# PlasmaControl/spectrogram-enhancement

Measured on AMD Instinct MI355X. Metric: spectrograms/s (STFT+VAE-denoise fwd) at 1/2/4/8 GPUs; PSNR vs CPU ref, higher is better.
Workload: dtype fp16; 1 GPU; BASELINE config 5 per GPU: end-to-end STFT -> SVD -> autoencoder-denoise inference stream, 16,512-sample fp16 shots -> specgr 128x128 (256 hann / hop 128) -> denoiseSignal default -> 3-layer conv AE (16/32/64, 5x5) fp16 forward -> fp16 reconstructions (32,768 B per shot); shots_per_launch=2048, samples=16512, stft_dtype=fp32, svd_dtype=fp32 (fp64 small algebra), ae_dtype=fp16, parallelism=shot-sharded x1, streams_per_gpu=2

## Files before the change

spectrogram-enhancement_amd/csrc/runtime.hip:

```cpp
#include "runtime.hpp"

#include <algorithm>
#include <atomic>
#include <cstdlib>
#include <cstring>
#include <mutex>
#include <string>

#include "specenh.h"

namespace specenh {
namespace {

struct VariantName {
  const char* name;
  int dflt;
};
constexpr VariantName kVariants[V_COUNT] = {
    {"CONVT_PAIR", 0},      {"PATCH_NO_WL", 0},      {"PATCH_NO_K5", 0},
    {"PATCH_WSPLIT", -1},   {"CONV_NO_S2", 0},       {"CONV_NO_PATCH", 0},
    {"CONV_NO_C1MFMA", 0},  {"CONV_NO_NARROW", 0},   {"WGRAD_GENERIC", 0},
    {"WGRAD_NO_CO1", 0},    {"WGRAD_PERPHASE", 0},   {"SVD_GRAM_TILES", 0},
    {"TAIL_TILES", 0},      {"DECODER_UNFUSED", 0},  {"SVD_NO_TOP1", 0},
    {"CONV_NO_ROWS", 0},    {"CONVT_NO_ROWS", 0},    {"CONV1_NO_ROWS", 0},
    {"ENCODER_UNFUSED", 0},  {"STFT_NO_HOLD", 0},    {"D3_MAP", 0},
    {"ENC2_WPE2", 0},        {"CONVT_SHARED_RING", 0}, {"SVD_RECON_VALU", 0},
    {"ROWS_SHORT_LEAD", 0},  {"SVD_GRAM_F32", 0},
    {"SVD_RECON_BLOCKS", 0}, {"CONVT_PG", 0}, {"SVD_GZ_ROWS", 0}, {"EIG_SPLIT", 0}, {"CO1_VALU", 0},
    {"C1_MASK_MFMA", 1}, {"S2_MIN_NT", 2}, {"PATCH_MIN_WG", 512}, {"WGRAD_WG", 1024}, {"WGRAD_C1_TILES", 4},
    {"EIG_GRID", 32}, {"ROWS_BANDS", -1}, {"CONVT_STORE8", 0},
    {"CONV_ROWS_SCHED", 1}, {"ENC2_SCHED", 1},
};

std::atomic<int> g_variant[V_COUNT];
std::once_flag g_variant_once;

void init_variants() {
  for (int i = 0; i < V_COUNT; ++i) {
    int v = kVariants[i].dflt;
    std::string env = std::string("SPECENH_") + kVariants[i].name;
    if (const char* s = std::getenv(env.c_str()); s && *s) v = std::atoi(s);
    g_variant[i].store(v, std::memory_order_relaxed);
  }
}

int variant_index(const char* name) {
  if (!name) return -1;
  if (std::strncmp(name, "SPECENH_", 8) == 0) name += 8;
  for (int i = 0; i < V_COUNT; ++i)
    if (std::strcmp(name, kVariants[i].name) == 0) return i;
  return -1;
}

constexpr int kMaxDevices = 64;
std::atomic<int> g_cus[kMaxDevices];

constexpr int kRing = 256;
thread_local const void* g_ring[kRing];
thread_local long long g_launches = 0;

thread_local std::string g_last_error;

}

int set_error(int code, const std::string& msg) {
  g_last_error = msg;
  return code;
}

int variant(Variant v) {
  std::call_once(g_variant_once, init_variants);
  return g_variant[v].load(std::memory_order_relaxed);
}

int device_cus() {
  int dev = 0;
  if (hipGetDevice(&dev) != hipSuccess || dev < 0 || dev >= kMaxDevices) return 256;
  int c = g_cus[dev].load(std::memory_order_relaxed);
  if (c > 0) return c;
  if (hipDeviceGetAttribute(&c, hipDeviceAttributeMultiprocessorCount, dev) != hipSuccess || c <= 0)
    c = 256;
  g_cus[dev].store(c, std::memory_order_relaxed);
  return c;
}

hipError_t allow_lds(LdsOptIn& site, std::initializer_list<const void*> kernels, int bytes) {
  static_assert(sizeof(site.done) / sizeof(site.done[0]) == kMaxDevices, "one flag per device");
  int dev = 0;
  hipError_t e = hipGetDevice(&dev);
  if (e != hipSuccess) return e;
  const bool known = dev >= 0 && dev < kMaxDevices;
  if (known && site.done[dev].load(std::memory_order_acquire)) return hipSuccess;
  for (const void* k : kernels) {
    hipFuncAttributes fa{};
    e = hipFuncGetAttributes(&fa, k);
    if (e != hipSuccess) return e;
    e = hipFuncSetAttribute(k, hipFuncAttributeMaxDynamicSharedMemorySize,
                            std::min(bytes, 160 * 1024 - (int)fa.sharedSizeBytes));
    if (e != hipSuccess) return e;
  }
  if (known) site.done[dev].store(true, std::memory_order_release);
  return hipSuccess;
}

hipError_t resident_slots(ResidentSlots& site, const void* kernel, int threads, int lds_bytes,
                          long long* slots) {
  static_assert(sizeof(site.per_cu) / sizeof(site.per_cu[0]) == kMaxDevices, "one count per device");
  int dev = 0;
  hipError_t e = hipGetDevice(&dev);
  if (e != hipSuccess) return e;
  const bool known = dev >= 0 && dev < kMaxDevices;
  int pc = known ? site.per_cu[dev].load(std::memory_order_relaxed) : 0;
  if (pc == 0) {
    e = hipOccupancyMaxActiveBlocksPerMultiprocessor(&pc, kernel, threads, (size_t)lds_bytes);
// ... 83 lines not shown
```

spectrogram-enhancement_amd/csrc/runtime.hpp:

```cpp
#pragma once

#include <hip/hip_runtime.h>

#include <atomic>
#include <initializer_list>
#include <string>

#include "specenh.h"

namespace specenh {

int set_error(int code, const std::string& msg);

inline int ilog2i(int n) {
  int l = 0;
  while ((1 << l) < n) ++l;
  return l;
}

enum Variant : int {
  V_CONVT_PAIR = 0,
  V_PATCH_NO_WL,
  V_PATCH_NO_K5,
  V_PATCH_WSPLIT,
  V_CONV_NO_S2,
  V_CONV_NO_PATCH,
  V_CONV_NO_C1MFMA,
  V_CONV_NO_NARROW,
  V_WGRAD_GENERIC,
  V_WGRAD_NO_CO1,
  V_WGRAD_PERPHASE,
  V_SVD_GRAM_TILES,
  V_TAIL_TILES,
  V_DECODER_UNFUSED,
  V_SVD_NO_TOP1,
  V_CONV_NO_ROWS,
  V_CONVT_NO_ROWS,
  V_CONV1_NO_ROWS,
  V_ENCODER_UNFUSED,
  V_STFT_NO_HOLD,
  V_D3_MAP,
  V_ENC2_WPE2,
  V_CONVT_SHARED_RING,
  V_SVD_RECON_VALU,
  V_ROWS_SHORT_LEAD,
  V_SVD_GRAM_F32,
  V_SVD_RECON_BLOCKS,
  V_CONVT_PG,
  V_SVD_GZ_ROWS,
  V_EIG_SPLIT,
  V_CO1_VALU,
  V_C1_MASK_MFMA,
  V_S2_MIN_NT,
  V_PATCH_MIN_WG,
  V_WGRAD_WG,
  V_WGRAD_C1_TILES,
  V_EIG_GRID,
  V_ROWS_BANDS,
  V_CONVT_STORE8,
  V_CONV_ROWS_SCHED,
  V_ENC2_SCHED,
  V_COUNT
};

int variant(Variant v);

int device_cus();

struct LdsOptIn {
  std::atomic<bool> done[64];
};
hipError_t allow_lds(LdsOptIn& site, std::initializer_list<const void*> kernels, int bytes);

struct ResidentSlots {
  std::atomic<int> per_cu[64];
};
hipError_t resident_slots(ResidentSlots& site, const void* kernel, int threads, int lds_bytes,
                          long long* slots);

template <typename F>
auto with_half_type(int dtype, F&& f) {
  return dtype == SPECENH_DTYPE_F16 ? f(_Float16{}) : f(__bf16{});
}

void note_launch(const void* kernel);

}

#define SPECENH_LAUNCH(K, ...)                                        \
  do {                                                                \
    ::specenh::note_launch(reinterpret_cast<const void*>(&K));        \
    hipLaunchKernelGGL(K, __VA_ARGS__);                               \
  } while (0)
```

spectrogram-enhancement_amd/csrc/svd_denoise.hip:

```cpp
#include <hip/hip_runtime.h>

#include <algorithm>
#include <cmath>
#include <cstdlib>
#include <string>
#include <vector>

#include "fft_common.hpp"
#include "specenh.h"
#include "runtime.hpp"
#include "wave.hpp"

namespace specenh {

typedef float f32x16 __attribute__((ext_vector_type(16)));

struct XView {
  const float* base;
  long long batch_stride;
  long long sk, si;
};

__global__ __launch_bounds__(256) void gram_kernel(XView x, int K, int r, float* G,
                                                   int ntiles_side) {
// ... 1499 lines not shown
      const int klen = RP / KS;
      for (int t = wave; t < 2 * NT * KS; t += 4) {
        const int tile = t % (2 * NT), part = t / (2 * NT);
        const int rt = tile & 1, ct = tile >> 1;
        const float* a_p = sX + (16 * rt + cl) * PX + part * klen + kr;
        const float* b_p = sV + (part * klen + kr) * PV + 16 * ct + cl;
        f4 acc = f4{0.f, 0.f, 0.f, 0.f}, acc2 = f4{0.f, 0.f, 0.f, 0.f};
        int k = 0;
        for (; k + 32 <= klen; k += 32) {
          float av[8], bv[8];
#pragma unroll
          for (int q = 0; q < 8; ++q) {
            av[q] = a_p[k + 4 * q];
            bv[q] = b_p[(k + 4 * q) * PV];
          }
#pragma unroll
          for (int q = 0; q < 8; q += 2) {
            acc = __builtin_amdgcn_mfma_f32_16x16x4f32(av[q], bv[q], acc, 0, 0, 0);
            acc2 = __builtin_amdgcn_mfma_f32_16x16x4f32(av[q + 1], bv[q + 1], acc2, 0, 0, 0);
          }
        }
        for (; k < klen; k += 4)
          acc = __builtin_amdgcn_mfma_f32_16x16x4f32(a_p[k], b_p[k * PV], acc, 0, 0, 0);
        acc += acc2;
        float* yp = sY + part * RB * PY + (16 * rt + 4 * kr) * PY + 16 * ct + cl;
#pragma unroll
        for (int j = 0; j < 4; ++j) yp[j * PY] = acc[j];
      }
    }
    lds_barrier();
    if constexpr (KS == 2) {
      for (int e = tid; e < RB * KPP; e += 256) {
        const int row = e / KPP, c = e % KPP;
        sY[row * PY + c] += sY[RB * PY + row * PY + c];
      }
      lds_barrier();
    }
    for (int t = wave; t < 2 * nit; t += 4) {
      const int rt = t & 1, it = t >> 1;
      const float* y_p = sY + (16 * rt + cl) * PY + kr;
      const float* v_p = sV + (16 * it + cl) * PV + kr;
      f4 acc = f4{0.f, 0.f, 0.f, 0.f};
#pragma unroll
      for (int k = 0; k < KPP; k += 4)
        acc = TRANS ? __builtin_amdgcn_mfma_f32_16x16x4f32(v_p[k], y_p[k], acc, 0, 0, 0)
                    : __builtin_amdgcn_mfma_f32_16x16x4f32(y_p[k], v_p[k], acc, 0, 0, 0);
#pragma unroll
      for (int j = 0; j < 4; ++j) {
        const int row = TRANS ? 16 * rt + cl : 16 * rt + 4 * kr + j;
        const int col = TRANS ? 16 * it + 4 * kr + j : 16 * it + cl;
        if (row < rows && col < r) {
          const float v = complement ? sX[row * PX + col] - acc[j] : acc[j];
          Ob[(long long)(k0 + row) * osk + (long long)col * osi] = to_out<TO>(v);
        }
      }
    }
  };
  fetch(stA, blk0 * RB, min(RB, Kr - blk0 * RB));
  fetch(stB, (blk0 + 1) * RB, blk0 + 1 < blk1 ? min(RB, Kr - (blk0 + 1) * RB) : 0);
  for (int blk = blk0; blk < blk1; blk += 2) {
    block(blk, stA);
    if (blk + 1 < blk1) block(blk + 1, stB);
  }
}

#ifndef SPECENH_TOP1_SWZ
#define SPECENH_TOP1_SWZ 1
#endif
namespace top1 {
constexpr int N = 128;
constexpr int LD = N + 4;
constexpr int MAX_ROUNDS = 24;
constexpr int ZP = SPECENH_TOP1_SWZ ? N + 8 : N;
__host__ __device__ constexpr int zt(int p, int k) {
  return p * ZP + k + (SPECENH_TOP1_SWZ ? 4 * (k >> 6) : 0);
}
__device__ __forceinline__ int ppos(int i) { return SPECENH_TOP1_SWZ ? i ^ ((i >> 3) & 7) : i; }
__device__ __forceinline__ int xz_chunk(int g, int j) {
  if (SPECENH_TOP1_SWZ)
    return 2 * (j >> 1) + (g >> 2) + 4 * ((j & 1) + 2 * ((g >> 1) & 1)) + 16 * (g & 1);
  return 8 * (g & 1) + (g >> 1) + 16 * (j & 1) + 4 * (j >> 1);
}
constexpr size_t LDS_BYTES = (size_t)N * LD * 4 + 4 * ZP * 4 + N * 4 * 4 + 4 * N * 4 * 4 + 64 * 8;

__device__ __forceinline__ void chol4(const double (&M)[4][4], double (&L)[4][4], double (&rinv)[4]) {
#pragma unroll
  for (int j = 0; j < 4; ++j) {
    double d = M[j][j];
#pragma unroll
    for (int l = 0; l < j; ++l) d = fma(-L[j][l], L[j][l], d);
    const bool live = d > 1e-20 * M[j][j] && d > 0.0;
    rinv[j] = live ? rsq64<1>(d) : 0.0;
    L[j][j] = 0.0;
#pragma unroll
    for (int k = j + 1; k < 4; ++k) {
      double s = M[k][j];
#pragma unroll
      for (int l = 0; l < j; ++l) s = fma(-L[k][l], L[j][l], s);
      L[k][j] = s * rinv[j];
      L[j][k] = 0.0;
    }
  }
}

__device__ __forceinline__ void solve_row(const double (&L)[4][4], const double (&rinv)[4],
                                          const double (&y)[4], double (&z)[4]) {
#pragma unroll
  for (int j = 0; j < 4; ++j) {
    double s = y[j];
#pragma unroll
    for (int l = 0; l < j; ++l) s = fma(-z[l], L[j][l], s);
    z[j] = s * rinv[j];
  }
}

__device__ __forceinline__ void jacobi4(float (&A)[4][4], float (&Q)[4][4]) {
#pragma unroll
  for (int a = 0; a < 4; ++a)
#pragma unroll
    for (int b = 0; b < 4; ++b) Q[a][b] = a == b ? 1.f : 0.f;
  for (int sweep = 0; sweep < 6; ++sweep) {
    float off = 0.f, dg = 0.f;
#pragma unroll
    for (int a = 0; a < 4; ++a) {
      dg = fmaf(A[a][a], A[a][a], dg);
#pragma unroll
      for (int b = a + 1; b < 4; ++b) off = fmaf(A[a][b], A[a][b], off);
    }
    if (!(off > 1e-14f * dg)) break;
#pragma unroll
    for (int pr = 0; pr < 6; ++pr) {
      const int p = pr < 3 ? 0 : (pr < 5 ? 1 : 2);
      const int q = pr < 3 ? pr + 1 : (pr < 5 ? pr - 1 : 3);
      const float apq = A[p][q];
      if (apq == 0.f) continue;
      const float tau = 0.5f * (A[q][q] - A[p][p]) * __builtin_amdgcn_rcpf(apq);
      const float t = copysignf(__builtin_amdgcn_rcpf(fabsf(tau) + __builtin_amdgcn_sqrtf(fmaf(tau, tau, 1.f))), tau);
      const float c = __builtin_amdgcn_rsqf(fmaf(t, t, 1.f)), s = t * c;
#pragma unroll
      for (int k = 0; k < 4; ++k) {
        const float akp = A[k][p], akq = A[k][q];
        A[k][p] = c * akp - s * akq;
        A[k][q] = s * akp + c * akq;
        const float qkp = Q[k][p], qkq = Q[k][q];
        Q[k][p] = c * qkp - s * qkq;
        Q[k][q] = s * qkp + c * qkq;
      }
#pragma unroll
      for (int k = 0; k < 4; ++k) {
        const float apk = A[p][k], aqk = A[q][k];
        A[p][k] = c * apk - s * aqk;
        A[q][k] = s * apk + c * aqk;
      }
    }
  }
}

template <int NV>
__device__ __forceinline__ void bsum128(double (&v)[NV], double* sR) {
  const int tid = threadIdx.x, w = tid >> 6;
  if (w < 2) {
#pragma unroll
    for (int j = 0; j < NV; ++j) v[j] = wave_sum_dpp(v[j]);
    if ((tid & 63) == 0)
#pragma unroll
      for (int j = 0; j < NV; ++j) sR[w * NV + j] = v[j];
  }
  lds_barrier();
#pragma unroll
  for (int j = 0; j < NV; ++j) v[j] = sR[j] + sR[NV + j];
}

template <int NV>
__device__ __forceinline__ void gram_sums(const float* sY, const float* sZt, const float* sU,
                                          double* sRed) {
  const int t = threadIdx.x, j = t >> 3, c = t & 7;
  double s = 0.0;
  if (j < NV) {
    const int n = j % 10, src = j / 10;
    const int a = (int)((0x3221110000ULL >> (4 * n)) & 15);
    const int b = (int)((0x3323213210ULL >> (4 * n)) & 15);
#pragma unroll
    for (int i = 0; i < 16; ++i) {
      const int row = SPECENH_TOP1_SWZ ? 8 * i + c : 16 * c + i;
      const float va = src == 0 ? sY[4 * row + a] : (src == 1 ? sZt[zt(a, row)] : sU[4 * row + a]);
      const float vb = src == 0 ? sY[4 * row + b] : (src == 1 ? sZt[zt(b, row)] : sU[4 * row + b]);
      s = fma((double)va, (double)vb, s);
    }
  }
  s += dpp<0xB1, false>(s);
  s += dpp<0x4E, false>(s);
  s += dpp<0x141, false>(s);
  if (c == 0 && j < NV) sRed[j] = s;
  lds_barrier();
}

__device__ __forceinline__ void sym4(const double* p, double (&M)[4][4]) {
  int n = 0;
#pragma unroll
  for (int a = 0; a < 4; ++a)
#pragma unroll
    for (int c = a; c < 4; ++c) {
      M[a][c] = M[c][a] = p[n];
      ++n;
    }
}
}

template <typename TO>
__global__ __launch_bounds__(256, 2) void top1_kernel(XView x, int Kr, int r, float tolv,
                                                       int* flags, TO* out, long long ob,
                                                       long long osk, long long osi,
                                                       long long batch, long long* phase_clk) {
  using namespace top1;
#ifdef SPECENH_TOP1_STATS
  long long tacc[8], tlast;
#define T1_MARK(slot)                                      \
  do {                                                     \
    const long long now_ = __builtin_amdgcn_s_memtime();   \
    tacc[slot] += now_ - tlast;                            \
    tlast = now_;                                          \
  } while (0)
#else
#define T1_MARK(slot) \
  do {                \
  } while (0)
#endif
  extern __shared__ __attribute__((aligned(16))) unsigned char smem[];
  float* sX = reinterpret_cast<float*>(smem);
  float* sZt = sX + N * LD;
  float* sU = sZt + 4 * ZP;
  float* sP = sU + 4 * N;
  double* sR = reinterpret_cast<double*>(sP + 16 * N);
  double* vd = reinterpret_cast<double*>(sP);
  double* ud = vd + N;
  double* hd = ud + N;
  const int tid = threadIdx.x, lane = tid & 63, w = tid >> 6;
#ifdef SPECENH_TOP1_STATS
  for (int q = 0; q < 8; ++q) tacc[q] = 0;
  tlast = __builtin_amdgcn_s_memtime();
#endif
  const long long b = blockIdx.x;
  if (b >= batch) return;
  const float* X = x.base + b * x.batch_stride;

  double fro = 0.0;
  if (x.si == 1) {
    constexpr int NLD = N * N / 4 / 256;
    float4 v[NLD];
#pragma unroll
    for (int u = 0; u < NLD; ++u) {
      const int e = tid + 256 * u, k = e >> 5, i = 4 * (e & 31);
      v[u] = (k < Kr && i < r) ? *reinterpret_cast<const float4*>(X + (long long)k * x.sk + i)
                               : make_float4(0.f, 0.f, 0.f, 0.f);
    }
#pragma unroll
    for (int u = 0; u < NLD; ++u) {
      const int e = tid + 256 * u, k = e >> 5, i = 4 * (e & 31);
      *reinterpret_cast<float4*>(sX + k * LD + i) = v[u];
      fro += (double)v[u].x * v[u].x + (double)v[u].y * v[u].y + (double)v[u].z * v[u].z +
             (double)v[u].w * v[u].w;
    }
  } else {
    for (int e = tid; e < N * N / 4; e += 256) {
      const int i = e >> 5, k = 4 * (e & 31);
      const float4 v = (k < Kr && i < r)
                           ? *reinterpret_cast<const float4*>(X + (long long)i * x.si + k)
                           : make_float4(0.f, 0.f, 0.f, 0.f);
      sX[k * LD + i] = v.x;
// ... 199 lines not shown
    {
      double S[4][4];
      sym4(sR, S);
      chol4(S, L, ri);
    }
    if (tid < N) {
#pragma unroll
      for (int p = 0; p < 4; ++p) yd[p] = y[p];
      solve_row(L, ri, yd, zd);
#pragma unroll
      for (int p = 0; p < 4; ++p) sZt[zt(p, tid)] = (float)zd[p];
    }
    lds_barrier();
    T1_MARK(3);
  }
  auto Xv = [&]() {
    const int k = tid & (N - 1), h = tid >> 7;
    const float* xr = sX + k * LD + 64 * h;
    const double* vv = vd + 64 * h;
    double s0 = 0.0, s1 = 0.0;
#pragma unroll 4
    for (int j = 0; j < 16; ++j) {
      const float4 x4 = *reinterpret_cast<const float4*>(xr + 4 * j);
      const double2 v01 = *reinterpret_cast<const double2*>(vv + 4 * j);
      const double2 v23 = *reinterpret_cast<const double2*>(vv + 4 * j + 2);
      s0 = fma((double)x4.x, v01.x, s0);
      s1 = fma((double)x4.y, v01.y, s1);
      s0 = fma((double)x4.z, v23.x, s0);
      s1 = fma((double)x4.w, v23.y, s1);
    }
    if (h) hd[k] = s0 + s1;
    lds_barrier();
    if (!h) ud[k] = (s0 + s1) + hd[k];
    lds_barrier();
  };
  lds_barrier();
  Xv();
  {
    const int i = tid & (N - 1), h = tid >> 7;
    double s0 = 0.0, s1 = 0.0;
#pragma unroll 8
    for (int kk = 0; kk < 64; kk += 2) {
      const int k = 64 * h + kk;
      s0 = fma((double)sX[k * LD + i], ud[k], s0);
      s1 = fma((double)sX[(k + 1) * LD + i], ud[k + 1], s1);
    }
    if (h) hd[i] = s0 + s1;
    lds_barrier();
    const double w = h ? 0.0 : (s0 + s1) + hd[i];
    double nn[1] = {w * w};
    bsum128<1>(nn, sR + 40);
    if (!h) vd[i] = nn[0] > 0.0 ? w * rsq64<1>(nn[0]) : 0.0;
    lds_barrier();
  }
  Xv();
  T1_MARK(5);
#ifdef SPECENH_TOP1_STATS
  if (flags && tid == 0) flags[b] = bad + 2 * t_used;
#else
  if (flags && tid == 0) flags[b] = bad;
#endif
  TO* Ob = out + b * ob;
  if (osi == 1) {
    for (int e = tid; e < Kr * (r / 4); e += 256) {
      const int k = e / (r / 4), i = 4 * (e % (r / 4));
      const float4 xv = *reinterpret_cast<const float4*>(sX + k * LD + i);
      const double2 v01 = *reinterpret_cast<const double2*>(vd + i);
      const double2 v23 = *reinterpret_cast<const double2*>(vd + i + 2);
      const double u = ud[k];
      TO* o = Ob + (long long)k * osk + i;
      o[0] = to_out<TO>((float)fma(-u, v01.x, (double)xv.x));
      o[1] = to_out<TO>((float)fma(-u, v01.y, (double)xv.y));
      o[2] = to_out<TO>((float)fma(-u, v23.x, (double)xv.z));
      o[3] = to_out<TO>((float)fma(-u, v23.y, (double)xv.w));
    }
  } else {
    for (int e = tid; e < r * (Kr / 4); e += 256) {
      const int i = e / (Kr / 4), k = 4 * (e % (Kr / 4));
      const double vi = vd[i];
      TO* o = Ob + (long long)i * osi + k;
#pragma unroll
      for (int c = 0; c < 4; ++c)
        o[c] = to_out<TO>((float)fma(-ud[k + c], vi, (double)sX[(k + c) * LD + i]));
    }
  }
  T1_MARK(6);
#ifdef SPECENH_TOP1_STATS
  if (phase_clk && tid == 0)
    for (int q = 0; q < 8; ++q) phase_clk[b * 8 + q] = tacc[q];
#endif
#undef T1_MARK
}



__device__ __forceinline__ void gram64_one(XView x, int K, int r, double* G, int nts,
                                           long long b, int tile) {
  __shared__ double sa[16][65], sb[16][65];
  int t = tile, ti = 0;
  while (t >= nts - ti) {
    t -= nts - ti;
    ++ti;
  }
  const int tj = ti + t;
  const float* X = x.base + b * x.batch_stride;
  const int tid = threadIdx.x, tx = tid & 15, ty = tid >> 4;
  double acc[4][4];
#pragma unroll
  for (int i = 0; i < 4; ++i)
#pragma unroll
    for (int j = 0; j < 4; ++j) acc[i][j] = 0.0;
  for (int k0 = 0; k0 < K; k0 += 16) {
    for (int idx = tid; idx < 16 * 64; idx += 256) {
      int kk, c;
      if (x.si == 1) {
        kk = idx >> 6;
        c = idx & 63;
      } else {
        c = idx >> 4;
        kk = idx & 15;
      }
      const int k = k0 + kk, ci = ti * 64 + c, cj = tj * 64 + c;
      sa[kk][c] = (k < K && ci < r) ? (double)X[(long long)k * x.sk + (long long)ci * x.si] : 0.0;
      sb[kk][c] = (k < K && cj < r) ? (double)X[(long long)k * x.sk + (long long)cj * x.si] : 0.0;
    }
    __syncthreads();
#pragma unroll 4
    for (int kk = 0; kk < 16; ++kk) {
      double av[4], bv[4];
#pragma unroll
      for (int i = 0; i < 4; ++i) {
        av[i] = sa[kk][ty * 4 + i];
        bv[i] = sb[kk][tx * 4 + i];
      }
#pragma unroll
      for (int i = 0; i < 4; ++i)
#pragma unroll
        for (int j = 0; j < 4; ++j) acc[i][j] = fma(av[i], bv[j], acc[i][j]);
    }
    __syncthreads();
  }
  double* Gb = G + b * (long long)r * r;
#pragma unroll
  for (int i = 0; i < 4; ++i)
#pragma unroll
    for (int j = 0; j < 4; ++j) {
      const int row = ti * 64 + ty * 4 + i, col = tj * 64 + tx * 4 + j;
      if (row < r && col < r) {
        Gb[(long long)row * r + col] = acc[i][j];
        Gb[(long long)col * r + row] = acc[i][j];
      }
    }
}

__global__ __launch_bounds__(256) void gram64_kernel(XView x, int K, int r, double* G, int nts,
                                                     const int* only, long long nmat) {
  for (long long b = blockIdx.y; b < nmat; b += gridDim.y) {
    if (only && !only[b]) continue;
    gram64_one(x, K, r, G, nts, b, blockIdx.x);
    __syncthreads();
  }
}

__device__ __forceinline__ void tridiag_one(double* G, int n, double* dg, double* eg,
                                            double* taug, long long b) {
  __shared__ double sv[256], sw[256], red[4];
// ... 699 lines not shown
  const EigLayout L = eig_layout(r);
  const long long ch = L.chunk(batch);
  char* w = (char*)workspace;
  double* G64 = (double*)w;
  double* dd = G64 + ch * (long long)r * r;
  double* ee = dd + ch * r;
  double* tau = ee + ch * r;
  double* Z = tau + ch * r;
  double* fac = Z + ch * (long long)r * L.ld;
  int* kinfo = (int*)(fac + 3 * ch * (long long)r * L.ld);
  int* ranges = kinfo + 2 * ch;
  int* num = ranges + 2 * ch;
  double* med = (double*)(((uintptr_t)(num + ch) + 7) & ~(uintptr_t)7);
  const Oriented o = orient(A, m, n, a_stride);
  XView xv = o.xv;
  const int Kr = o.Kr;
  const long long osk = o.osk, osi = o.osi;
  const long long ob = (long long)m * n;
  const size_t osz = dtype_size(odt);
  const int nts64 = (r + 63) / 64, ntri64 = nts64 * (nts64 + 1) / 2;
  const double beta = (double)r / (double)std::max(m, n);
  const double omega = ((0.0 + 0.56 * std::pow(beta, 3.0)) + -0.95 * std::pow(beta, 2.0)) +
                       1.82 * std::pow(beta, 1.0) + 1.43 * std::pow(beta, 0.0);
  for (long long b0 = 0; b0 < batch; b0 += ch) {
    const long long nb = std::min(ch, batch - b0);
    xv.base = A + b0 * a_stride;
    const int* on = only ? only + b0 : nullptr;
    void* ob0 = static_cast<char*>(out) + (size_t)(b0 * ob) * osz;
    const long long gcap = variant(V_EIG_GRID) > 0 ? variant(V_EIG_GRID) : 2LL * device_cus();
    const unsigned gm = on ? (unsigned)std::min<long long>(nb, gcap) : (unsigned)nb;
    const bool merged_fits = (long long)r * Kr <= 128LL * 128;
    if (on && opt_mode < 0 && merged_fits && SPECENH_EIG_MERGED && variant(V_EIG_SPLIT) == 0) {
      const hipError_t e = with_out_type(odt, [&](auto t) {
        return launch_eig_fallback_t<decltype(t)>(xv, Kr, r, G64, nts64, dd, ee, tau, lo, hi, Z,
                                                  fac, L.ld, kinfo, ob0, ob, osk, osi, on, nb, gm,
                                                  st);
      });
      if (e != hipSuccess) return set_error(SPECENH_EHIP, std::string("eigen fallback: ") + hipGetErrorString(e));
      continue;
    }
    SPECENH_LAUNCH(gram64_kernel, dim3(ntri64, gm), dim3(256), 0, st, xv, Kr, r, G64, nts64, on,
                   nb);
    SPECENH_LAUNCH(tridiag_kernel, dim3(gm), dim3(256), 0, st, G64, r, dd, ee, tau, on, nb);
    const int* rg = nullptr;
    if (opt_mode >= 0) {
      SPECENH_LAUNCH(optimal_rank_kernel, dim3((unsigned)nb), dim3(64), 0, st, dd, ee, r,
                         omega, num, med);
      SPECENH_LAUNCH(optimal_ranges_kernel, dim3((unsigned)((nb + 255) / 256)), dim3(256), 0,
                         st, num, nb, r, opt_mode, ranges, bad);
      if (num_out && hipMemcpyAsync(num_out + b0, num, (size_t)nb * 4, hipMemcpyDeviceToDevice,
                                    st) != hipSuccess)
        return set_error(SPECENH_EHIP, "num_sing copy");
      if (med_out && hipMemcpyAsync(med_out + b0, med, (size_t)nb * 8, hipMemcpyDeviceToDevice,
                                    st) != hipSuccess)
        return set_error(SPECENH_EHIP, "median copy");
      rg = ranges;
    }
    SPECENH_LAUNCH(eigvec_kernel, dim3(gm), dim3(256), 0, st, G64, dd, ee, tau, r, lo, hi, rg,
                   Z, fac, L.ld, kinfo, on, nb);
    if (hipGetLastError() != hipSuccess) return set_error(SPECENH_EHIP, "eigen path launch");
    const hipError_t e = with_out_type(odt, [&](auto t) {
      return launch_recon_eig_t<decltype(t)>(xv, Kr, r, Z, L.ld, kinfo, ob0, ob, osk, osi, nb, st,
                                             on);
    });
    if (e != hipSuccess) return set_error(SPECENH_EHIP, std::string("recon: ") + hipGetErrorString(e));
  }
  return SPECENH_OK;
}

bool top1_fits(const float* A, int m, int n, long long a_stride) {
  return m <= top1::N && n <= top1::N && m % 4 == 0 && n % 4 == 0 && a_stride % 4 == 0 &&
         ((uintptr_t)A & 15) == 0;
}

template <typename TO>
hipError_t launch_top1_t(const float* A, long long batch, int m, int n, long long a_stride,
                         int* flags, void* out, hipStream_t st, long long* phase_clk) {
  static LdsOptIn lds_site;
  const hipError_t attr =
      allow_lds(lds_site, {(const void*)top1_kernel<TO>}, (int)top1::LDS_BYTES);
  if (attr != hipSuccess) return attr;
  const auto [xv, Kr, osk, osi] = orient(A, m, n, a_stride);
  const int r = std::min(m, n);
  for (long long b0 = 0; b0 < batch; b0 += 1LL << 30) {
    const long long nb = std::min<long long>(1LL << 30, batch - b0);
    XView xb = xv;
    xb.base = A + b0 * a_stride;
    SPECENH_LAUNCH(top1_kernel<TO>, dim3((unsigned)nb), dim3(256), top1::LDS_BYTES, st, xb, Kr,
                   r, 5e-6f, flags + b0, reinterpret_cast<TO*>(out) + b0 * (long long)m * n,
                   (long long)m * n, osk, osi, nb, phase_clk ? phase_clk + 8 * b0 : nullptr);
  }
  return hipGetLastError();
}

void resolve_slice(int r, int start, int stop, int& lo, int& hi) {
  if (start < 0) start = 0;
  if (stop > r) stop = r;
  lo = std::min(start, r);
  hi = stop < 0 ? std::max(stop + r, 0) : stop;
  if (hi < lo) hi = lo;
}

int range_path(int r, int lo, int hi, int& K) {
  K = 0;
  if (hi <= lo || (lo == 0 && hi == r)) return 0;
  K = hi == r ? lo : hi;
  return (K <= PMAX - 8 && std::max(8, ((K + 7 + 7) / 8) * 8) <= std::max(8, (r / 8) * 8) &&
          ((r / 8) * 8 >= K))
             ? 1
             : 2;
}

struct SubspaceWs {
  size_t G, V, theta, flags, flags2, eig, total;
};
SubspaceWs subspace_ws(long long batch, long long r, int K) {
  SubspaceWs w{};
  w.V = (size_t)(batch * r * r) * sizeof(float);
  w.theta = (size_t)(batch * r * r + batch * r * K) * sizeof(float);
  w.total = (size_t)(batch * r * r + batch * r * K + batch * K) * sizeof(float);
  if (r > EIG_MAXN) return w;
  w.flags = (w.total + 255) / 256 * 256;
  w.flags2 = w.flags + (size_t)batch * 4;
  w.eig = (w.flags + 2 * (size_t)batch * 4 + 255) / 256 * 256;
  w.total = w.eig + eig_layout((int)r).bytes(batch);
  return w;
}
SubspaceWs top1_ws(long long batch, int r, int path, int K) {
  if (path == 1) return subspace_ws(batch, r, K);
  SubspaceWs w{};
  w.flags = eig_layout(r).bytes(batch);
  w.total = w.flags + batch * 4 + 256;
  return w;
}
}

extern "C" {

size_t specenh_svd_workspace_bytes(long long batch, int m, int n, int kmax) {
  const long long r = std::min(m, n);
  if (batch <= 0 || r <= 0) return 16;
  if (kmax > PMAX - 8 && r <= EIG_MAXN) return eig_layout((int)r).bytes(batch);
  return subspace_ws(batch, r, kmax).total;
}

size_t specenh_svd_denoise_workspace_bytes(long long batch, int m, int n, int start, int stop) {
  if (batch <= 0 || m <= 0 || n <= 0) return 16;
  const int r = std::min(m, n);
  int lo, hi, K;
  resolve_slice(r, start, stop, lo, hi);
  switch (range_path(r, lo, hi, K)) {
    case 1: return specenh_svd_workspace_bytes(batch, m, n, K);
    case 2:
      if (r > EIG_MAXN) return 16;
      return lo == 1 && hi == r ? top1_ws(batch, r, 2, K).total : eig_layout(r).bytes(batch);
    default: return 16;
  }
}

int specenh_svd_denoise(const float* A, long long batch, int m, int n, long long a_stride,
                        int start, int stop, float* out, void* workspace, void* stream) {
  return specenh_svd_denoise_ex(A, batch, m, n, a_stride, start, stop, out, SPECENH_DTYPE_F32,
                                workspace, stream);
}

int specenh_svd_denoise_ex(const float* A, long long batch, int m, int n, long long a_stride,
                           int start, int stop, void* out, int out_dtype, void* workspace,
                           void* stream) {
  if (out_dtype != SPECENH_DTYPE_F32 && out_dtype != SPECENH_DTYPE_F16 &&
      out_dtype != SPECENH_DTYPE_BF16)
    return set_error(SPECENH_EINVAL, "svd output dtype must be f32, bf16 or f16");
  if (batch < 0 || m <= 0 || n <= 0) return set_error(SPECENH_EINVAL, "bad matrix shape");
  if (batch == 0) return SPECENH_OK;
// ... 143 lines not shown
```

Baseline: 2.090 million spectrograms/s.

## Keep SVD top-1 input matrix in registers instead of LDS

Adds a top1_kernel_reg variant in which each thread holds its 128x128 slice of the input matrix in VGPRs across all subspace-iteration rounds, so the matrix is no longer staged in LDS. Cross-lane reductions use DPP and permlane swaps, and a small padded LDS area covers the remaining data. The cut in LDS use is meant to allow several workgroups per CU and to remove LDS reads of X on every round. The cost is heavy register pressure (launch bounds of 256 threads with 4 WGs) and possible spills, and the path only applies to unit-stride, aligned outputs, with an env variable to fall back to the old kernel.

```diff
diff --git a/spectrogram-enhancement_amd/csrc/runtime.hip b/spectrogram-enhancement_amd/csrc/runtime.hip
--- a/spectrogram-enhancement_amd/csrc/runtime.hip
+++ b/spectrogram-enhancement_amd/csrc/runtime.hip
@@ -29,7 +29,7 @@
     {"SVD_RECON_BLOCKS", 0}, {"CONVT_PG", 0}, {"SVD_GZ_ROWS", 0}, {"EIG_SPLIT", 0}, {"CO1_VALU", 0},
     {"C1_MASK_MFMA", 1}, {"S2_MIN_NT", 2}, {"PATCH_MIN_WG", 512}, {"WGRAD_WG", 1024}, {"WGRAD_C1_TILES", 4},
     {"EIG_GRID", 32}, {"ROWS_BANDS", -1}, {"CONVT_STORE8", 0},
-    {"CONV_ROWS_SCHED", 1}, {"ENC2_SCHED", 1},
+    {"CONV_ROWS_SCHED", 1}, {"ENC2_SCHED", 1}, {"SVD_TOP1_LDS", 0},
 };
 
 std::atomic<int> g_variant[V_COUNT];
diff --git a/spectrogram-enhancement_amd/csrc/runtime.hpp b/spectrogram-enhancement_amd/csrc/runtime.hpp
--- a/spectrogram-enhancement_amd/csrc/runtime.hpp
+++ b/spectrogram-enhancement_amd/csrc/runtime.hpp
@@ -60,6 +60,7 @@
   V_CONVT_STORE8,
   V_CONV_ROWS_SCHED,
   V_ENC2_SCHED,
+  V_SVD_TOP1_LDS,
   V_COUNT
 };
 
diff --git a/spectrogram-enhancement_amd/csrc/svd_denoise.hip b/spectrogram-enhancement_amd/csrc/svd_denoise.hip
--- a/spectrogram-enhancement_amd/csrc/svd_denoise.hip
+++ b/spectrogram-enhancement_amd/csrc/svd_denoise.hip
@@ -1605,6 +1605,9 @@
   return 8 * (g & 1) + (g >> 1) + 16 * (j & 1) + 4 * (j >> 1);
 }
 constexpr size_t LDS_BYTES = (size_t)N * LD * 4 + 4 * ZP * 4 + N * 4 * 4 + 4 * N * 4 * 4 + 64 * 8;
+__host__ __device__ constexpr int uoff(int k) { return 4 * (k + (k >> 4)); }
+constexpr int UW = uoff(N);
+constexpr size_t REG_LDS_BYTES = 4 * ZP * 4 + UW * 4 + 4 * N * 4 * 4 + 64 * 8;
 
 __device__ __forceinline__ void chol4(const double (&M)[4][4], double (&L)[4][4], double (&rinv)[4]) {
 #pragma unroll
@@ -1680,8 +1683,8 @@
 }
 
 template <int NV>
-__device__ __forceinline__ void bsum128(double (&v)[NV], double* sR) {
-  const int tid = threadIdx.x, w = tid >> 6;
+__device__ __forceinline__ void bsum128(double (&v)[NV], double* sR, int tid = threadIdx.x) {
+  const int w = tid >> 6;
   if (w < 2) {
 #pragma unroll
     for (int j = 0; j < NV; ++j) v[j] = wave_sum_dpp(v[j]);
@@ -1694,10 +1697,10 @@
   for (int j = 0; j < NV; ++j) v[j] = sR[j] + sR[NV + j];
 }
 
-template <int NV>
+template <int NV, bool UP = false>
 __device__ __forceinline__ void gram_sums(const float* sY, const float* sZt, const float* sU,
-                                          double* sRed) {
-  const int t = threadIdx.x, j = t >> 3, c = t & 7;
+                                          double* sRed, int t = threadIdx.x) {
+  const int j = t >> 3, c = t & 7;
   double s = 0.0;
   if (j < NV) {
     const int n = j % 10, src = j / 10;
@@ -1706,8 +1709,9 @@
 #pragma unroll
     for (int i = 0; i < 16; ++i) {
       const int row = SPECENH_TOP1_SWZ ? 8 * i + c : 16 * c + i;
-      const float va = src == 0 ? sY[4 * row + a] : (src == 1 ? sZt[zt(a, row)] : sU[4 * row + a]);
-      const float vb = src == 0 ? sY[4 * row + b] : (src == 1 ? sZt[zt(b, row)] : sU[4 * row + b]);
+      const int ur = UP ? uoff(row) : 4 * row;
+      const float va = src == 0 ? sY[4 * row + a] : (src == 1 ? sZt[zt(a, row)] : sU[ur + a]);
+      const float vb = src == 0 ? sY[4 * row + b] : (src == 1 ? sZt[zt(b, row)] : sU[ur + b]);
       s = fma((double)va, (double)vb, s);
     }
   }
@@ -2073,6 +2077,419 @@
 #pragma unroll
       for (int c = 0; c < 4; ++c)
         o[c] = to_out<TO>((float)fma(-ud[k + c], vi, (double)sX[(k + c) * LD + i]));
+    }
+  }
+  T1_MARK(6);
+#ifdef SPECENH_TOP1_STATS
+  if (phase_clk && tid == 0)
+    for (int q = 0; q < 8; ++q) phase_clk[b * 8 + q] = tacc[q];
+#endif
+#undef T1_MARK
+}
+
+namespace top1 {
+template <int CTRL, typename T>
+__device__ __forceinline__ T rs_dpp(bool up, T lo, T hi) {
+  const T keep = up ? hi : lo, send = up ? lo : hi;
+  return keep + dpp<CTRL, false>(send);
+}
+__device__ __forceinline__ float rs_swap32(float lo, float hi) {
+  const auto s = __builtin_amdgcn_permlane32_swap(__float_as_uint(lo), __float_as_uint(hi), false, false);
+  return __uint_as_float(s[0]) + __uint_as_float(s[1]);
+}
+__device__ __forceinline__ float rs_swap16(float lo, float hi) {
+  const auto s = __builtin_amdgcn_permlane16_swap(__float_as_uint(lo), __float_as_uint(hi), false, false);
+  return __uint_as_float(s[0]) + __uint_as_float(s[1]);
+}
+__device__ __forceinline__ double rs_swap32(double lo, double hi) {
+  const unsigned long long l = __double_as_longlong(lo), h = __double_as_longlong(hi);
+  const auto s0 = __builtin_amdgcn_permlane32_swap((unsigned)l, (unsigned)h, false, false);
+  const auto s1 = __builtin_amdgcn_permlane32_swap((unsigned)(l >> 32), (unsigned)(h >> 32), false, false);
+  return __longlong_as_double(((unsigned long long)s1[0] << 32) | s0[0]) +
+         __longlong_as_double(((unsigned long long)s1[1] << 32) | s0[1]);
+}
+__device__ __forceinline__ double rs_swap16(double lo, double hi) {
+  const unsigned long long l = __double_as_longlong(lo), h = __double_as_longlong(hi);
+  const auto s0 = __builtin_amdgcn_permlane16_swap((unsigned)l, (unsigned)h, false, false);
+  const auto s1 = __builtin_amdgcn_permlane16_swap((unsigned)(l >> 32), (unsigned)(h >> 32), false, false);
+  return __longlong_as_double(((unsigned long long)s1[0] << 32) | s0[0]) +
+         __longlong_as_double(((unsigned long long)s1[1] << 32) | s0[1]);
+}
+template <typename TO>
+struct alignas(4 * sizeof(TO)) Out4 {
+  TO v[4];
+};
+}
+#ifndef SPECENH_TOP1_REG_WGS
+#define SPECENH_TOP1_REG_WGS 4
+#endif
+
+template <typename TO>
+__global__ __launch_bounds__(256, SPECENH_TOP1_REG_WGS) void top1_kernel_reg(XView x, int Kr, int r, float tolv,
+                                                           int* flags, TO* out, long long ob,
+                                                           long long osk, long long batch,
+                                                           long long* phase_clk) {
+  using namespace top1;
+#ifdef SPECENH_TOP1_STATS
+  long long tacc[8], tlast;
+#define T1_MARK(slot)                                      \
+  do {                                                     \
+    const long long now_ = __builtin_amdgcn_s_memtime();   \
+    tacc[slot] += now_ - tlast;                            \
+    tlast = now_;                                          \
+  } while (0)
+#else
+#define T1_MARK(slot) \
+  do {                \
+  } while (0)
+#endif
+  __shared__ __attribute__((aligned(16))) unsigned char smem[REG_LDS_BYTES];
+  float* sZt = reinterpret_cast<float*>(smem);
+  float* sU = sZt + 4 * ZP;
+  float* sP = sU + UW;
+  double* sR = reinterpret_cast<double*>(sP + 16 * N);
+  double* vd = reinterpret_cast<double*>(sP);
+  double* ud = vd + N;
+  double* wd = ud + N;
+  int tid = threadIdx.x, lane, w, a, c, i0;
+  bool c3, c2, c1, c0;
+  auto lane_map = [&]() {
+    lane = tid & 63, w = tid >> 6, a = tid >> 4, c = tid & 15;
+    c3 = c & 8, c2 = c & 4, c1 = c & 2, c0 = c & 1;
+    i0 = 64 * (lane >> 5) + 4 * c + 2 * ((lane >> 4) & 1);
+  };
+  lane_map();
+  auto fresh_map = [&]() {
+    asm volatile("" : "+v"(tid));
+    lane_map();
+  };
+#ifdef SPECENH_TOP1_STATS
+  for (int q = 0; q < 8; ++q) tacc[q] = 0;
+  tlast = __builtin_amdgcn_s_memtime();
+#endif
+  const long long b = blockIdx.x;
+  if (b >= batch) return;
+  const float* X = x.base + b * x.batch_stride;
+
+  float4 xr[8][2];
+#pragma unroll
+  for (int m = 0; m < 8; ++m)
+#pragma unroll
+    for (int h = 0; h < 2; ++h) {
+      const int k = a + 16 * m, i = 4 * c + 64 * h;
+      xr[m][h] = (k < Kr && i < r) ? *reinterpret_cast<const float4*>(X + (long long)k * x.sk + i)
+                                   : make_float4(0.f, 0.f, 0.f, 0.f);
+    }
+  auto pin_x = [&]() {
+#pragma unroll
+    for (int m = 0; m < 8; ++m)
+#pragma unroll
+      for (int h = 0; h < 2; ++h)
+        asm volatile("" : "+v"(xr[m][h].x), "+v"(xr[m][h].y), "+v"(xr[m][h].z), "+v"(xr[m][h].w));
+  };
+  if (tid < N)
+#pragma unroll
+    for (int p = 0; p < 4; ++p)
+      sZt[zt(p, tid)] = tid < r ? (p == 0 ? 1.f : hash_unit(tid, p)) : 0.f;
+  lds_barrier();
+  T1_MARK(0);
+
+  for (int t = 1;; ++t) {
+    fresh_map();
+    {
+      float acc[32];
+#pragma unroll
+      for (int q = 0; q < 32; ++q) acc[q] = 0.f;
+#pragma unroll
+      for (int h = 0; h < 2; ++h)
+#pragma unroll
+        for (int p = 0; p < 4; ++p) {
+          const float4 zv = *reinterpret_cast<const float4*>(sZt + zt(p, 4 * c + 64 * h));
+#pragma unroll
+          for (int m = 0; m < 8; ++m) {
+            const float4 xv = xr[m][h];
+            float s = acc[4 * m + p];
+            s = fmaf(xv.x, zv.x, s);
+            s = fmaf(xv.y, zv.y, s);
+            s = fmaf(xv.z, zv.z, s);
+            s = fmaf(xv.w, zv.w, s);
+            acc[4 * m + p] = s;
+          }
+        }
+      float a16[16], a8[8], a4[4], a2[2];
+      fresh_map();
+#pragma unroll
+      for (int q = 0; q < 16; ++q) a16[q] = rs_dpp<0x128>(c3, acc[q], acc[16 + q]);
+#pragma unroll
+      for (int q = 0; q < 8; ++q) a8[q] = rs_dpp<0x141>(c2, a16[q], a16[8 + q]);
+#pragma unroll
+      for (int q = 0; q < 4; ++q) a4[q] = rs_dpp<0x4E>(c1, a8[q], a8[4 + q]);
+#pragma unroll
+      for (int q = 0; q < 2; ++q) a2[q] = rs_dpp<0xB1>(c0, a4[q], a4[2 + q]);
+      *reinterpret_cast<float2*>(sU + uoff(a + 16 * (c >> 1)) + 2 * (c & 1)) = make_float2(a2[0], a2[1]);
+    }
+    if (t == 1) {
+      double fro = 0.0;
+#pragma unroll
+      for (int m = 0; m < 8; ++m)
+#pragma unroll
+        for (int h = 0; h < 2; ++h) {
+          const float4 v = xr[m][h];
+          fro += (double)v.x * v.x + (double)v.y * v.y + (double)v.z * v.z + (double)v.w * v.w;
+        }
+#pragma unroll
+      for (int m = 32; m >= 1; m >>= 1) fro += __shfl_xor(fro, m);
+      if (lane == 0) sR[32 + w] = fro;
+      pin_x();
+    }
+    lds_barrier();
+    T1_MARK(1);
+    {
+      float acc[32];
+      fresh_map();
+#pragma unroll
+      for (int q = 0; q < 32; ++q) acc[q] = 0.f;
+#pragma unroll
+      for (int m = 0; m < 8; ++m) {
+        const float4 uv = *reinterpret_cast<const float4*>(sU + uoff(a + 16 * m));
+#pragma unroll
+        for (int h = 0; h < 2; ++h) {
+          const float xs[4] = {xr[m][h].x, xr[m][h].y, xr[m][h].z, xr[m][h].w};
+#pragma unroll
+          for (int e = 0; e < 4; ++e) {
+            const int q = 4 * (4 * h + e);
+            acc[q + 0] = fmaf(xs[e], uv.x, acc[q + 0]);
+            acc[q + 1] = fmaf(xs[e], uv.y, acc[q + 1]);
+            acc[q + 2] = fmaf(xs[e], uv.z, acc[q + 2]);
+            acc[q + 3] = fmaf(xs[e], uv.w, acc[q + 3]);
+          }
+        }
+      }
+      float a16[16], a8[8];
+      fresh_map();
+#pragma unroll
+      for (int q = 0; q < 16; ++q) a16[q] = rs_swap32(acc[q], acc[16 + q]);
+#pragma unroll
+      for (int q = 0; q < 8; ++q) a8[q] = rs_swap16(a16[q], a16[8 + q]);
+      float* dst = sP + w * 4 * N;
+      *reinterpret_cast<float4*>(dst + 4 * ppos(i0)) = make_float4(a8[0], a8[1], a8[2], a8[3]);
+      *reinterpret_cast<float4*>(dst + 4 * ppos(i0 + 1)) = make_float4(a8[4], a8[5], a8[6], a8[7]);
+    }
+    lds_barrier();
+    if (tid < N) {
+      const int pt = ppos(tid);
+      float4 s = *reinterpret_cast<const float4*>(sP + 4 * pt);
+#pragma unroll
+      for (int ww = 1; ww < 4; ++ww) {
+        const float4 o = *reinterpret_cast<const float4*>(sP + ww * 4 * N + 4 * pt);
+        s.x += o.x; s.y += o.y; s.z += o.z; s.w += o.w;
+      }
+      *reinterpret_cast<float4*>(sP + 4 * tid) = s;
+    }
+    lds_barrier();
+    T1_MARK(2);
+    const bool check = t >= 2 && (t <= 4 || t % 2 == 0 || t == MAX_ROUNDS);
+    if (check) {
+      gram_sums<30, true>(sP, sZt, sU, sR, tid);
+      double L[4][4], ri[4];
+      {
+        double M[4][4];
+        sym4(sR + 10, M);
+        chol4(M, L, ri);
+      }
+      double H[4][4];
+      sym4(sR + 20, H);
+      double W[4][4];
+      float C[4][4];
+#pragma unroll
+      for (int cc = 0; cc < 4; ++cc) {
+#pragma unroll
+        for (int aa = 0; aa < 4; ++aa) {
+          double s = H[aa][cc];
+#pragma unroll
+          for (int l = 0; l < aa; ++l) s = fma(-L[aa][l], W[l][cc], s);
+          W[aa][cc] = s * ri[aa];
+        }
+      }
+#pragma unroll
+      for (int cc = 0; cc < 4; ++cc) {
+        double col[4];
+#pragma unroll
+        for (int aa = 0; aa < 4; ++aa) {
+          double s = W[cc][aa];
+#pragma unroll
+          for (int l = 0; l < aa; ++l) s = fma(-L[aa][l], col[l], s);
+          col[aa] = s * ri[aa];
+        }
+#pragma unroll
+        for (int aa = cc; aa < 4; ++aa) C[aa][cc] = C[cc][aa] = (float)col[aa];
+      }
+      if (tid == 0) {
+#pragma unroll
+        for (int l = 1; l < 4; ++l)
+#pragma unroll
+          for (int aa = 0; aa < l; ++aa) sR[46 + l * (l - 1) / 2 + aa] = L[l][aa];
+#pragma unroll
+        for (int n = 0; n < 4; ++n) sR[52 + n] = ri[n];
+      }
+      float Q[4][4];
+      jacobi4(C, Q);
+      float th1f = C[0][0], th2f = -3.0e38f, qt[4] = {Q[0][0], Q[1][0], Q[2][0], Q[3][0]};
+#pragma unroll
+      for (int aa = 1; aa < 4; ++aa) {
+        const bool gt = C[aa][aa] > th1f;
+        th2f = fmaxf(th2f, gt ? th1f : C[aa][aa]);
+        th1f = gt ? C[aa][aa] : th1f;
+#pragma unroll
+        for (int cc = 0; cc < 4; ++cc) qt[cc] = gt ? Q[cc][aa] : qt[cc];
+      }
+      lds_barrier();
+      double q1[4];
+#pragma unroll
+      for (int aa = 3; aa >= 0; --aa) {
+        double s = qt[aa];
+#pragma unroll
+        for (int l = aa + 1; l < 4; ++l) s = fma(-sR[46 + l * (l - 1) / 2 + aa], q1[l], s);
+        q1[aa] = s * sR[52 + aa];
+      }
+      double vi = 0.0, gv = 0.0;
+      if (tid < N) {
+        const float4 y4 = *reinterpret_cast<const float4*>(sP + 4 * tid);
+        const float y[4] = {y4.x, y4.y, y4.z, y4.w};
+#pragma unroll
+        for (int p = 0; p < 4; ++p) {
+          vi = fma((double)sZt[zt(p, tid)], q1[p], vi);
+          gv = fma((double)y[p], q1[p], gv);
+        }
+      }
+      double rs[3] = {gv * vi, vi * vi, gv * gv};
+      bsum128<3>(rs, sR + 40, tid);
+      const double tr = (sR[32] + sR[33]) + (sR[34] + sR[35]);
+      const double vv = fmax(rs[1], 1e-300);
+      const double th1 = rs[0] / vv;
+      const double res2 = fmax(rs[2] - th1 * rs[0], 0.0) / vv;
+      const double th2 = fmin((double)th2f, th1);
+      const double rest = fmax(tr - th1, 1e-4 * fmax(tr, 0.0));
+      const double f = fmin(1.0, rest / fmax(th1, 1e-300));
+      float tol = tolv;
+      asm volatile("" : "+v"(tol));
+      const bool conv = sqrt(fmax(th1, 0.0) * res2) * f <= (double)tol * (th1 - th2) * sqrt(rest);
+      if (conv || t >= MAX_ROUNDS) {
+#ifdef SPECENH_TOP1_STATS
+        if (flags && tid == 0) flags[b] = (conv ? 0 : 1) + 2 * t;
+#else
+        if (flags && tid == 0) flags[b] = conv ? 0 : 1;
+#endif
+        if (tid < N) vd[tid] = vi * rsq64<1>(vv);
+        T1_MARK(4);
+        break;
+      }
+      T1_MARK(4);
+    } else {
+      gram_sums<10, true>(sP, sZt, sU, sR, tid);
+    }
+    double L[4][4], ri[4], yd[4], zd[4];
+    {
+      double S[4][4];
+      sym4(sR, S);
+      chol4(S, L, ri);
+    }
+    if (tid < N) {
+      const float4 y4 = *reinterpret_cast<const float4*>(sP + 4 * tid);
+      yd[0] = y4.x, yd[1] = y4.y, yd[2] = y4.z, yd[3] = y4.w;
+      solve_row(L, ri, yd, zd);
+#pragma unroll
+      for (int p = 0; p < 4; ++p) sZt[zt(p, tid)] = (float)zd[p];
+    }
+    lds_barrier();
+    T1_MARK(3);
+  }
+  auto Xv = [&]() {
+    double s[8];
+    pin_x();
+    fresh_map();
+#pragma unroll
+    for (int m = 0; m < 8; ++m) s[m] = 0.0;
+#pragma unroll
+    for (int h = 0; h < 2; ++h) {
+      const double2 v01 = *reinterpret_cast<const double2*>(vd + 4 * c + 64 * h);
+      const double2 v23 = *reinterpret_cast<const double2*>(vd + 4 * c + 64 * h + 2);
+#pragma unroll
+      for (int m = 0; m < 8; ++m) {
+        const float4 x4 = xr[m][h];
+        s[m] = fma((double)x4.x, v01.x, s[m]);
+        s[m] = fma((double)x4.y, v01.y, s[m]);
+        s[m] = fma((double)x4.z, v23.x, s[m]);
+        s[m] = fma((double)x4.w, v23.y, s[m]);
+      }
+    }
+    double s4[4], s2[2];
+#pragma unroll
+    for (int q = 0; q < 4; ++q) s4[q] = rs_dpp<0x128>(c3, s[q], s[4 + q]);
+#pragma unroll
+    for (int q = 0; q < 2; ++q) s2[q] = rs_dpp<0x141>(c2, s4[q], s4[2 + q]);
+    double s1 = rs_dpp<0x4E>(c1, s2[0], s2[1]);
+    s1 += dpp<0xB1, false>(s1);
+    if (!c0) ud[a + 16 * (c >> 1)] = s1;
+    lds_barrier();
+  };
+  lds_barrier();
+  Xv();
+  {
+    double s[8];
+    pin_x();
+    fresh_map();
+#pragma unroll
+    for (int q = 0; q < 8; ++q) s[q] = 0.0;
+#pragma unroll
+    for (int m = 0; m < 8; ++m) {
+      const double u = ud[a + 16 * m];
+#pragma unroll
+      for (int h = 0; h < 2; ++h) {
+        const float4 x4 = xr[m][h];
+        s[4 * h + 0] = fma((double)x4.x, u, s[4 * h + 0]);
+        s[4 * h + 1] = fma((double)x4.y, u, s[4 * h + 1]);
+        s[4 * h + 2] = fma((double)x4.z, u, s[4 * h + 2]);
+        s[4 * h + 3] = fma((double)x4.w, u, s[4 * h + 3]);
+      }
+    }
+    double s4[4], s2[2];
+#pragma unroll
+    for (int q = 0; q < 4; ++q) s4[q] = rs_swap32(s[q], s[4 + q]);
+#pragma unroll
+    for (int q = 0; q < 2; ++q) s2[q] = rs_swap16(s4[q], s4[2 + q]);
+    *reinterpret_cast<double2*>(wd + w * N + i0) = make_double2(s2[0], s2[1]);
+    lds_barrier();
+    const double wv = tid < N ? (wd[tid] + wd[N + tid]) + (wd[2 * N + tid] + wd[3 * N + tid]) : 0.0;
+    double nn[1] = {wv * wv};
+    bsum128<1>(nn, sR + 40, tid);
+    if (tid < N) vd[tid] = nn[0] > 0.0 ? wv * rsq64<1>(nn[0]) : 0.0;
+    lds_barrier();
+  }
+  Xv();
+  T1_MARK(5);
+  TO* Ob = out + b * ob;
+  pin_x();
+  fresh_map();
+#pragma unroll
+  for (int h = 0; h < 2; ++h) {
+    const int i = 4 * c + 64 * h;
+    const double2 v01 = *reinterpret_cast<const double2*>(vd + i);
+    const double2 v23 = *reinterpret_cast<const double2*>(vd + i + 2);
+#pragma unroll
+    for (int m = 0; m < 8; ++m) {
+      const int k = a + 16 * m;
+      const double u = ud[k];
+      const float4 xv = xr[m][h];
+      float f[4] = {(float)fma(-u, v01.x, (double)xv.x), (float)fma(-u, v01.y, (double)xv.y),
+                    (float)fma(-u, v23.x, (double)xv.z), (float)fma(-u, v23.y, (double)xv.w)};
+      Out4<TO> o;
+#pragma unroll
+      for (int e = 0; e < 4; ++e) {
+        asm volatile("" : "+v"(f[e]));
+        o.v[e] = to_out<TO>(f[e]);
+      }
+      if (k < Kr && i < r) *reinterpret_cast<Out4<TO>*>(Ob + (long long)k * osk + i) = o;
     }
   }
   T1_MARK(6);
@@ -2938,13 +3355,20 @@
   if (attr != hipSuccess) return attr;
   const auto [xv, Kr, osk, osi] = orient(A, m, n, a_stride);
   const int r = std::min(m, n);
+  const bool reg = xv.si == 1 && osi == 1 && ((uintptr_t)out % (4 * sizeof(TO))) == 0 &&
+                   variant(V_SVD_TOP1_LDS) == 0;
   for (long long b0 = 0; b0 < batch; b0 += 1LL << 30) {
     const long long nb = std::min<long long>(1LL << 30, batch - b0);
     XView xb = xv;
     xb.base = A + b0 * a_stride;
-    SPECENH_LAUNCH(top1_kernel<TO>, dim3((unsigned)nb), dim3(256), top1::LDS_BYTES, st, xb, Kr,
-                   r, 5e-6f, flags + b0, reinterpret_cast<TO*>(out) + b0 * (long long)m * n,
-                   (long long)m * n, osk, osi, nb, phase_clk ? phase_clk + 8 * b0 : nullptr);
+    TO* ob0 = reinterpret_cast<TO*>(out) + b0 * (long long)m * n;
+    long long* clk = phase_clk ? phase_clk + 8 * b0 : nullptr;
+    if (reg)
+      SPECENH_LAUNCH(top1_kernel_reg<TO>, dim3((unsigned)nb), dim3(256), 0, st, xb, Kr, r, 5e-6f,
+                     flags + b0, ob0, (long long)m * n, osk, nb, clk);
+    else
+      SPECENH_LAUNCH(top1_kernel<TO>, dim3((unsigned)nb), dim3(256), top1::LDS_BYTES, st, xb, Kr,
+                     r, 5e-6f, flags + b0, ob0, (long long)m * n, osk, osi, nb, clk);
   }
   return hipGetLastError();
 }
```

Result: faster. 2.130 million spectrograms/s, median of 6 (+1.9%).
